# vchuravy/NewtonKrylov.jl

Measured on AMD Instinct MI355X. Metric: Krylov matvecs/sec + achieved HBM GB/s, 2D Bratu 4096^2, higher is better.
Workload: dtype f64

## Files before the change

### newtonkrylov.jl_amd/csrc/nk_resident.hip

```cpp
#include <hip/hip_runtime.h>

#include <algorithm>
#include <cmath>
#include <cstdio>
#include <vector>

#include "nk_device.hpp"

namespace nk {
namespace {
constexpr int kResMax = 64;
constexpr int kResThreads = 256;
struct ResArgs {
    const double* V[kResMax + 1];
    double* q;
    double* vout;
    double* col;
    double* colh;
    const double* red_in;
    uint64_t* gran;
    int* err;
    int noxchg;
    int ntc;
    int nwc;
    int poll1;
    int strided;
    int mirror;
    uint64_t* tstamp;
    int senders;
    const double *ju, *jv, *jf0, *jaux;
    double jeps, jlam, jhx2, jhy2;
    int64_t jnx;
    int jv_on;
    int64_t n2;
    int np, red_len, rl;
    unsigned tag0, mb0, spin;
};

template <int RV>
struct ResState {
    dx2 r[RV];
};

__device__ __forceinline__ double res_exchange(const ResArgs& A, double part, int t, double* sh, unsigned& budget,
                                              unsigned* xdone) {
    const int tid = threadIdx.x, G = gridDim.x;
    const unsigned tag = A.tag0 + (unsigned)t;
    uint64_t* slot = A.gran + (size_t)(t & 1) * G * 2;
    if (tid == 0) {
        const uint64_t bits = (uint64_t)__double_as_longlong(part);
        __hip_atomic_store(slot + 2 * blockIdx.x, ((uint64_t)tag << 32) | (bits & 0xffffffffull), __ATOMIC_RELAXED,
                           __HIP_MEMORY_SCOPE_AGENT);
        __hip_atomic_store(slot + 2 * blockIdx.x + 1, ((uint64_t)tag << 32) | (bits >> 32), __ATOMIC_RELAXED,
                           __HIP_MEMORY_SCOPE_AGENT);
    }
    if (A.poll1) {
        const int w = tid >> 6, nw = A.poll1 >= 2 ? kResThreads / 64 : 1;
        if (w < nw) {
            for (int i = 0; i < w; ++i) __builtin_amdgcn_s_sleep(8);
            const int l = tid & 63;
            uint64_t w8[8];
            bool mine = false;
            for (;;) {
                if (nw > 1 && __hip_atomic_load(xdone, __ATOMIC_RELAXED, __HIP_MEMORY_SCOPE_WORKGROUP) == tag) break;
                bool ok = true;
#pragma unroll
                for (int j = 0; j < 4; ++j) {
                    const int bl = 64 * j + l;
                    if (bl < G) {
                        w8[2 * j] = __hip_atomic_load(slot + 2 * bl, __ATOMIC_RELAXED, __HIP_MEMORY_SCOPE_AGENT);
                        w8[2 * j + 1] = __hip_atomic_load(slot + 2 * bl + 1, __ATOMIC_RELAXED, __HIP_MEMORY_SCOPE_AGENT);
                        ok = ok && (unsigned)(w8[2 * j] >> 32) == tag && (unsigned)(w8[2 * j + 1] >> 32) == tag;
                    } else {
                        w8[2 * j] = w8[2 * j + 1] = 0;
                    }
                }
                if (__all(ok)) {
                    mine = true;
                    break;
                }
                if (budget == 0 || --budget == 0) {
                    __hip_atomic_store(A.err, 1, __ATOMIC_RELAXED, __HIP_MEMORY_SCOPE_SYSTEM);
                    mine = true;
                    break;
                }
                __builtin_amdgcn_s_sleep(2);
            }
            if (mine) {
                double p = 0.0;
#pragma unroll
                for (int j = 0; j < 4; ++j)
                    p += __longlong_as_double((long long)(((w8[2 * j + 1] & 0xffffffffull) << 32) | (w8[2 * j] & 0xffffffffull)));
                p = wave_sum(p);
                if (l == 0) {
                    sh[kShB] = p;
                    if (nw > 1) __hip_atomic_store(xdone, tag, __ATOMIC_RELAXED, __HIP_MEMORY_SCOPE_WORKGROUP);
                }
            }
        }
        __syncthreads();
        const double s1 = sh[kShB];
        if (A.mb0 == 0) return s1;
        const unsigned epoch = A.mb0 + (unsigned)t;
        if ((int)blockIdx.x < A.senders) mb_send(s1, epoch);
        __syncthreads();
        return mb_recv(epoch, sh);
    }
    double v = 0.0;
    if (tid < G) {
        const uint64_t* g = slot + 2 * tid;
        uint64_t lo = __hip_atomic_load(g, __ATOMIC_RELAXED, __HIP_MEMORY_SCOPE_AGENT);
        uint64_t hi = __hip_atomic_load(g + 1, __ATOMIC_RELAXED, __HIP_MEMORY_SCOPE_AGENT);
        while ((unsigned)(lo >> 32) != tag || (unsigned)(hi >> 32) != tag) {
            if (budget == 0 || --budget == 0) {
                __hip_atomic_store(A.err, 1, __ATOMIC_RELAXED, __HIP_MEMORY_SCOPE_SYSTEM);
                lo = hi = 0;
                break;
            }
            __builtin_amdgcn_s_sleep(1);
            lo = __hip_atomic_load(g, __ATOMIC_RELAXED, __HIP_MEMORY_SCOPE_AGENT);
            hi = __hip_atomic_load(g + 1, __ATOMIC_RELAXED, __HIP_MEMORY_SCOPE_AGENT);
        }
        v = __longlong_as_double((long long)(((hi & 0xffffffffull) << 32) | (lo & 0xffffffffull)));
    }
    __syncthreads();
    double s = block_sum<kResThreads>(v, sh);
    if (tid == 0) sh[kShB] = s;
    __syncthreads();
    s = sh[kShB];
    if (A.mb0 == 0) return s;
    const unsigned epoch = A.mb0 + (unsigned)t;
    if ((int)blockIdx.x < A.senders) mb_send(s, epoch);
    __syncthreads();
    return mb_recv(epoch, sh);
}

__device__ __forceinline__ dx2 res_jv_pair(const ResArgs& A, int64_t e, double& acc) {
    const int64_t p = 2 * e, nx = A.jnx;
    const int64_t i = p % nx;
    const dx2 vc = *reinterpret_cast<const dx2*>(A.jv + p), uc = __builtin_nontemporal_load(reinterpret_cast<const dx2*>(A.ju + p));
    const dx2 vu = *reinterpret_cast<const dx2*>(A.jv + p + nx), uu = *reinterpret_cast<const dx2*>(A.ju + p + nx);
    const dx2 vd = *reinterpret_cast<const dx2*>(A.jv + p - nx), ud = *reinterpret_cast<const dx2*>(A.ju + p - nx);
    const double vl = A.jv[p - 1], ul = A.ju[p - 1], vr = A.jv[p + 2], ur = A.ju[p + 2];
    const dx2 f0 = __builtin_nontemporal_load(reinterpret_cast<const dx2*>(A.jf0 + p));
    const dx2 ax = *reinterpret_cast<const dx2*>(A.jaux + p);
    const double eps = A.jeps;
    const double c0 = uc.x + eps * vc.x, c1 = uc.y + eps * vc.y;
    const double wl = i > 0 ? ul + eps * vl : 0.0;
    const double wr = i + 2 < nx ? ur + eps * vr : 0.0;
    const double u0 = uu.x + eps * vu.x, u1 = uu.y + eps * vu.y;
    const double d0 = ud.x + eps * vd.x, d1 = ud.y + eps * vd.y;
    const double l0 = ((c1 - 2.0 * c0) + wl) / A.jhx2 + ((u0 - 2.0 * c0) + d0) / A.jhy2;
    const double l1 = ((wr - 2.0 * c1) + c0) / A.jhx2 + ((u1 - 2.0 * c1) + d1) / A.jhy2;
    const double r0 = l0 + A.jlam * nk_exp(c0), r1 = l1 + A.jlam * nk_exp(c1);
    const dx2 val{(r0 - f0.x) / eps, (r1 - f0.y) / eps};
    acc = fma(ax.x, val.x, acc);
    acc = fma(ax.y, val.y, acc);
    return val;
}

template <int NTM>
__device__ __forceinline__ dx2 ldv(const dx2* p) {
    if constexpr (NTM == 1) return *p;
    else return __builtin_nontemporal_load(p);
}
template <int NTM>
__device__ __forceinline__ dx2 ldw(const dx2* p) {
    if constexpr (NTM == 2) return __builtin_nontemporal_load(p);
    else return *p;
}
template <int NTM>
__device__ __forceinline__ dx2 ldw_s(const dx2* p, int s, int nwc) {
#ifdef NK_KBENCH
    if (NTM != 2 && s >= nwc) return __builtin_nontemporal_load(p);
#else
    (void)s;
    (void)nwc;
#endif
    return ldw<NTM>(p);
}

template <int B>
struct ResPre {
    dx2 b[B], c[B];
};
template <int RV, int B, bool PRE, int NTM = 0>
__device__ __forceinline__ void res_prefetch(const ResArgs& A, ResPre<B>& P, int t, int64_t base, int64_t ss,
                                             bool rev = false) {
    if constexpr (PRE && RV >= B) {
        const int tid = threadIdx.x;
        const int s0 = (B == 4 && rev) ? RV + A.rl - 4 : 0;
        const dx2* vb = reinterpret_cast<const dx2*>(A.V[t]) + base + tid + s0 * ss;
        const dx2* wb = reinterpret_cast<const dx2*>(A.V[t + 1 < A.np ? t + 1 : t]) + base + tid + s0 * ss;
#pragma unroll
        for (int u = 0; u < B; ++u) {
            P.b[u] = ldv<NTM>(vb + u * ss);
            P.c[u] = ldw_s<NTM>(wb + u * ss, s0 + u, A.nwc);
        }
    }
}

template <int RV, int B, bool PRE, int NTM = 0, bool NTS = false, int LB = 4>
__device__ __forceinline__ double res_pass(const ResArgs& A, ResState<RV>& S, dx2* lq, int t, double mh, int64_t lo,
                                           int64_t hi, ResPre<B>& P, int64_t base, int64_t ss, bool rev = false) {
    const int tid = threadIdx.x;
    const bool next = t + 1 < A.np;
    const dx2* vb = reinterpret_cast<const dx2*>(A.V[t]) + base + tid;
    const dx2* wb = reinterpret_cast<const dx2*>(A.V[next ? t + 1 : t]) + base + tid;
    double acc = 0.0;
    auto upd = [&](dx2& a, const dx2 b, const dx2 c) {
        a.x = fma(mh, b.x, a.x);
        a.y = fma(mh, b.y, a.y);
        const dx2 p = next ? c : a;
        acc = fma(p.x, a.x, acc);
        acc = fma(p.y, a.y, acc);
    };
    auto regs = [&] {
        constexpr int NB = (RV + B - 1) / B;
#pragma unroll
        for (int bi = 0; bi < NB; ++bi) {
            const int s0 = bi * B;
            dx2 bv[B], cv[B];
            if (PRE && RV >= B && s0 == 0 && !(B == 4 && rev)) {
#pragma unroll
                for (int u = 0; u < B; ++u) {
                    bv[u] = P.b[u];
                    cv[u] = P.c[u];
                }
            } else {
#pragma unroll
                for (int u = 0; u < B; ++u) {
                    if (s0 + u < RV) {
                        bv[u] = ldv<NTM>(vb + (s0 + u) * ss);
                        cv[u] = ldw_s<NTM>(wb + (s0 + u) * ss, s0 + u, A.nwc);
                    }
                }
            }
#pragma unroll
            for (int u = 0; u < B; ++u)
                if (s0 + u < RV) upd(S.r[s0 + u], bv[u], cv[u]);
            __builtin_amdgcn_sched_barrier(0);
        }
    };
    const dx2* vl = vb + RV * ss;
    const dx2* wl = wb + RV * ss;
    const int rl = A.rl;
    auto lds = [&] {
        auto one4 = [&](int s, bool down) {
            dx2 bv[4], cv[4];
#pragma unroll
            for (int u = 0; u < 4; ++u) {
                bv[u] = ldv<NTM>(vl + (s + u) * ss);
                cv[u] = ldw_s<NTM>(wl + (s + u) * ss, RV + s + u, A.nwc);
            }
#pragma unroll
            for (int u0 = 0; u0 < 4; ++u0) {
                const int u = down ? 3 - u0 : u0;
                dx2 a = lq[(s + u) * kResThreads + tid];
                upd(a, bv[u], cv[u]);
                lq[(s + u) * kResThreads + tid] = a;
            }
        };
        auto one = [&](int s) {
            const dx2 b = ldv<NTM>(vl + s * ss);
            const dx2 cc = ldw_s<NTM>(wl + s * ss, RV + s, A.nwc);
            dx2 a = lq[s * kResThreads + tid];
            upd(a, b, cc);
            lq[s * kResThreads + tid] = a;
        };
        auto oneB = [&](int s) {
            dx2 bv[LB], cv[LB];
#pragma unroll
            for (int u = 0; u < LB; ++u) {
                bv[u] = ldv<NTM>(vl + (s + u) * ss);
                cv[u] = ldw_s<NTM>(wl + (s + u) * ss, RV + s + u, A.nwc);
            }
#pragma unroll
            for (int u = 0; u < LB; ++u) {
                dx2 a = lq[(s + u) * kResThreads + tid];
                upd(a, bv[u], cv[u]);
                lq[(s + u) * kResThreads + tid] = a;
            }
        };
        const int r4 = rl / 4 * 4;
        if (!rev && LB != 4) {
            const int rb = rl / LB * LB;
            for (int s = 0; s < rb; s += LB) oneB(s);
            for (int s = rb; s < r4; s += 4) one4(s, false);
            for (int s = r4; s < rl; ++s) one(s);
        } else if (!rev) {
            for (int s = 0; s < r4; s += 4) one4(s, false);
            for (int s = r4; s < rl; ++s) one(s);
        } else if (PRE && B == 4 && RV >= B) {
            {
                const int s = rl - 4;
#pragma unroll
                for (int u0 = 0; u0 < 4; ++u0) {
                    const int u = 3 - u0;
                    dx2 a = lq[(s + u) * kResThreads + tid];
                    upd(a, P.b[u], P.c[u]);
                    lq[(s + u) * kResThreads + tid] = a;
                }
            }
            int s = rl - 8;
            for (; s >= 0; s -= 4) one4(s, true);
            for (s += 3; s >= 0; --s) one(s);
        } else {
            for (int s = rl - 1; s >= r4; --s) one(s);
            for (int s = r4 - 4; s >= 0; s -= 4) one4(s, true);
        }
    };
    auto stream = [&] {
        dx2* q2 = reinterpret_cast<dx2*>(A.q);
        const dx2* v2 = reinterpret_cast<const dx2*>(A.V[t]);
        const dx2* w2 = reinterpret_cast<const dx2*>(A.V[next ? t + 1 : t]);
        auto ld = [](const dx2* p) {
            if constexpr (NTS) return __builtin_nontemporal_load(p);
            else return *p;
        };
        auto st = [](dx2* p, const dx2 v) {
            if constexpr (NTS) __builtin_nontemporal_store(v, p);
            else *p = v;
        };
        int64_t e = lo + (int64_t)(RV + rl) * kResThreads + tid;
        if constexpr (NTS) {
            const int64_t hc = std::min<int64_t>(hi, e - tid + (int64_t)A.ntc * kResThreads);
            for (; e + kResThreads < hc; e += 2 * kResThreads) {
                const int64_t e1 = e + kResThreads;
                dx2 a0 = ld(q2 + e), a1 = ld(q2 + e1);
                const dx2 b0 = __builtin_nontemporal_load(v2 + e), b1 = __builtin_nontemporal_load(v2 + e1);
                const dx2 c0 = w2[e], c1 = w2[e1];
                upd(a0, b0, c0);
                upd(a1, b1, c1);
                st(q2 + e, a0);
                st(q2 + e1, a1);
            }
        }
        for (; e + kResThreads < hi; e += 2 * kResThreads) {
            const int64_t e1 = e + kResThreads;
            dx2 a0 = ld(q2 + e), a1 = ld(q2 + e1);
            const dx2 b0 = __builtin_nontemporal_load(v2 + e), b1 = __builtin_nontemporal_load(v2 + e1);
            const dx2 c0 = ld(w2 + e), c1 = ld(w2 + e1);
            upd(a0, b0, c0);
            upd(a1, b1, c1);
            st(q2 + e, a0);
            st(q2 + e1, a1);
        }
        if (e < hi) {
            dx2 a0 = ld(q2 + e);
            const dx2 b0 = __builtin_nontemporal_load(v2 + e);
            const dx2 c0 = ld(w2 + e);
            upd(a0, b0, c0);
            st(q2 + e, a0);
        }
    };
    if (rev) lds();
    regs();
    if (!rev) lds();
    stream();
    return acc;
}

template <int RV, int B = (RV > 80 ? 6 : RV > 64 ? 4 : 8), bool PRE = false, bool JV = false, bool ALT = false,
          int NTM = 0, bool NTS = false, int LB = 4>
__global__ __launch_bounds__(kResThreads, 1) void k_mgs_res(ResArgs A) {
    extern __shared__ dx2 lq[];
    __shared__ double sh[kShN];
    __shared__ unsigned xdone;
    const int tid = threadIdx.x, G = gridDim.x;
    if (tid == 0) xdone = 0;
    const int64_t ns = (A.n2 + kResThreads - 1) / kResThreads;
    const int64_t lo = (int64_t)blockIdx.x * ns / G * kResThreads;
    const int64_t hi = std::min<int64_t>((int64_t)(blockIdx.x + 1) * ns / G * kResThreads, A.n2);
    int64_t base = A.strided ? (int64_t)blockIdx.x * kResThreads : lo;
    int64_t ss = A.strided ? (int64_t)G * kResThreads : kResThreads;
#ifdef NK_KBENCH
    if (A.mirror && (blockIdx.x & 1)) {
        base = hi - kResThreads;
        ss = -(int64_t)kResThreads;
    }
#endif
    ResState<RV> S;
    ResPre<B> P;
    double h;
    unsigned budget = A.spin;
    constexpr int xo = JV ? 1 : 0;
    if constexpr (JV) {
        double jacc = 0.0;
        constexpr int kJvStage = 16;
#pragma unroll
        for (int s0 = 0; s0 < RV; s0 += kJvStage) {
            const int m = RV - s0 < kJvStage ? RV - s0 : kJvStage;
#pragma unroll 4
            for (int u = 0; u < m; ++u) lq[u * kResThreads + tid] = res_jv_pair(A, base + (s0 + u) * ss + tid, jacc);
#pragma unroll
            for (int u = 0; u < kJvStage; ++u)
                if (s0 + u < RV) S.r[s0 + u] = lq[u * kResThreads + tid];
        }
#pragma unroll 4
        for (int s = 0; s < A.rl; ++s) lq[s * kResThreads + tid] = res_jv_pair(A, base + (RV + s) * ss + tid, jacc);
        res_prefetch<RV, B, PRE, NTM>(A, P, 0, base, ss);
        h = res_exchange(A, block_sum<kResThreads>(jacc, sh), 0, sh, budget, &xdone);
    } else {
        const dx2* qb = reinterpret_cast<const dx2*>(A.q) + base + tid;
#pragma unroll
        for (int s = 0; s < RV; ++s) S.r[s] = qb[s * ss];
        for (int s = 0; s < A.rl; ++s) lq[s * kResThreads + tid] = qb[(RV + s) * ss];
        res_prefetch<RV, B, PRE, NTM>(A, P, 0, base, ss);
        h = reduce_input(A.red_in, A.red_len, sh);
    }
    for (int t = 0; t < A.np; ++t) {
        if (blockIdx.x == 0 && tid == 0) {
            A.col[t] = h;
            if (A.colh) A.colh[t] = h;
        }
        const double acc = res_pass<RV, B, PRE, NTM, NTS, LB>(A, S, lq, t, -h, lo, hi, P, base, ss, ALT && (t & 1));
        if (t + 1 < A.np) res_prefetch<RV, B, PRE, NTM>(A, P, t + 1, base, ss, ALT && ((t + 1) & 1));
        const double part = block_sum<kResThreads>(acc, sh);
#ifdef NK_KBENCH
        if (A.tstamp && tid == 0) A.tstamp[((size_t)t * G + blockIdx.x) * 2] = wall_clock64();
        if (!A.noxchg) h = res_exchange(A, part, t + xo, sh, budget, &xdone);
        else __syncthreads();
        if (A.tstamp && tid == 0) A.tstamp[((size_t)t * G + blockIdx.x) * 2 + 1] = wall_clock64();
#else
        h = res_exchange(A, part, t + xo, sh, budget, &xdone);
#endif
    }
    if (blockIdx.x == 0 && tid == 0) {
        const double r = sqrt(h);
        A.col[A.np] = r;
        if (A.colh) A.colh[A.np] = r;
    }
    if (A.vout) {
        const double hn = sqrt(h);
        dx2* vw = reinterpret_cast<dx2*>(A.vout) + base + tid;
#pragma unroll
        for (int s = 0; s < RV; ++s) vw[s * ss] = dx2{S.r[s].x / hn, S.r[s].y / hn};
        for (int s = 0; s < A.rl; ++s) {
            const dx2 a = lq[s * kResThreads + tid];
            vw[(RV + s) * ss] = dx2{a.x / hn, a.y / hn};
        }
        return;
    }
    dx2* qw = reinterpret_cast<dx2*>(A.q) + base + tid;
#pragma unroll
    for (int s = 0; s < RV; ++s) qw[s * ss] = S.r[s];
    for (int s = 0; s < A.rl; ++s) qw[(RV + s) * ss] = lq[s * kResThreads + tid];
}

template <int RV, int B = (RV > 80 ? 6 : RV > 64 ? 4 : 8), bool PRE = false, bool JV = false, bool ALT = false,
          int NTM = 0, bool NTS = false, int LB = 4>
const char* go_res(dim3 g, dim3 b, size_t lds, hipStream_t s, const ResArgs& A) {
    hipLaunchKernelGGL((k_mgs_res<RV, B, PRE, JV, ALT, NTM, NTS, LB>), g, b, lds, s, A);
    static char name[80] = {};
    if (!name[0]) {
        auto tf = [](bool x) { return x ? "true" : "false"; };
        std::snprintf(name, sizeof name, "nk::k_mgs_res<%d, %d, %s, %s, %s, %d, %s, %d>", RV, B, tf(PRE), tf(JV), tf(ALT), NTM,
                      tf(NTS), LB);
    }
    return name;
}

template <int RV, int B = (RV > 80 ? 6 : RV > 64 ? 4 : 8), bool PRE = false, bool JV = false, bool ALT = false,
          int NTM = 0, bool NTS = false, int LB = 4>
bool res_attr(size_t lds) {
    return hipFuncSetAttribute(reinterpret_cast<const void*>(&k_mgs_res<RV, B, PRE, JV, ALT, NTM, NTS, LB>),
                               hipFuncAttributeMaxDynamicSharedMemorySize, (int)lds) == hipSuccess;
}
}

hipError_t resident_bind_mb(const MbInfo& m) { return hipMemcpyToSymbol(HIP_SYMBOL(g_mb), &m, sizeof(m)); }


int launch_mgs_sweep(nk_ctx* c, int64_t n, double* q, const double* const* V, int k, int np, Red in, double* col,
                     double* colh, int rv, double** vout, const ResJv* jin) {
    if (np < 1 || np > kResMax || (n & 1) || !c->res_ok) return 1;
#ifdef NK_KBENCH
    static const int jv_env = NK_TUNE("NK_RES_JV", 0);
    if (jin && (!jv_env || !vout || !*vout || jin->nx % 2 != 0)) return 1;
#else
    if (jin) return 1;
#endif
    if (c->comm && !c->mb_on) return 1;
    if (!c->res_gran) {
        int dev = 0, cus = 0, lds = 0;
        bool ok = hipGetDevice(&dev) == hipSuccess &&
                  hipDeviceGetAttribute(&cus, hipDeviceAttributeMultiprocessorCount, dev) == hipSuccess &&
                  hipDeviceGetAttribute(&lds, hipDeviceAttributeMaxSharedMemoryPerBlock, dev) == hipSuccess &&
                  cus >= 1 && cus <= kResThreads;
        if (ok) {
            c->res_blocks = std::max(1, cus / std::max(1, c->res_share));
            const int avail = lds - (int)(sizeof(double) * kShN) - 256;
            c->res_rl = std::max(0, avail / (int)(kResThreads * sizeof(dx2)));
            const size_t lmax = (size_t)c->res_rl * kResThreads * sizeof(dx2);
            ok = res_attr<0>(lmax) && res_attr<16>(lmax) && res_attr<25>(lmax) && res_attr<32>(lmax) && res_attr<48>(lmax) &&
                 res_attr<64>(lmax) && res_attr<89, 4, true>(lmax) && res_attr<89, 4, true, false, false, 0, true>(lmax);
#ifdef NK_KBENCH
            ok = ok && res_attr<89>(lmax) && res_attr<89, 4>(lmax) && res_attr<89, 6, false, true>(lmax) &&
                 res_attr<0, 8, false, true>(lmax) && res_attr<89, 6, false, false, true>(lmax) &&
                 res_attr<89, 6, false, false, false, 1>(lmax) && res_attr<89, 6, false, false, false, 2>(lmax) &&
                 res_attr<89, 6, false, false, false, 0, true>(lmax) && res_attr<89, 2, true>(lmax) &&
                 res_attr<89, 4, true, false, false, 0, false, 8>(lmax) &&
                 res_attr<89, 4, true, false, false, 0, false, 6>(lmax) && res_attr<89, 4, true, false, true>(lmax);
#endif
            int per_cu = 0;
            ok = ok && hipOccupancyMaxActiveBlocksPerMultiprocessor(
                           &per_cu, reinterpret_cast<const void*>(&k_mgs_res<89, 4, true>), kResThreads, lmax) == hipSuccess &&
                 per_cu >= 1;
        }
        ok = ok && hipMalloc(&c->res_gran, sizeof(uint64_t) * 4 * kResThreads) == hipSuccess;
        ok = ok && hipMemsetAsync(c->res_gran, 0, sizeof(uint64_t) * 4 * kResThreads, c->stream) == hipSuccess;
        ok = ok && hipHostMalloc(&c->res_err, sizeof(int), hipHostMallocMapped) == hipSuccess;
        if (ok) *c->res_err = 0;
        ok = ok && hipHostGetDevicePointer(reinterpret_cast<void**>(&c->res_err_dev), c->res_err, 0) == hipSuccess;
        if (!ok) {
            (void)hipGetLastError();
            c->res_ok = false;
            return 1;
        }
    }
    ResArgs A{};
    for (int t = 0; t < np; ++t) A.V[t] = V[t % k];
    A.V[np] = V[(np) % k];
    A.q = q;
    A.col = col;
    A.colh = colh;
    A.red_in = in.ptr;
    A.red_len = in.len;
    A.gran = c->res_gran;
    A.err = c->res_err_dev;
    A.n2 = n >> 1;
    A.np = np;
    static const int nts_env = NK_TUNE("NK_RES_NTS", 1);
    static const int pre_env = NK_TUNE("NK_RES_PRE", 1);
    int xv = -1;
    bool streamed = false;
    {
        const int64_t G = c->res_blocks, n2 = n >> 1;
        const int64_t ns = (n2 + kResThreads - 1) / kResThreads;
        const int64_t whole = ns / G - (n2 % kResThreads != 0 ? 1 : 0);
        if (whole < 1) return 1;
        const int slots = (int)std::min<int64_t>(whole, 1 << 20);
        static const int rl_env = NK_TUNE("NK_RES_RL", -1);
        static const int rv_env = NK_TUNE("NK_RES_RV", -1);
        int rl = std::min(slots, rl_env >= 0 ? std::min(rl_env, c->res_rl) : c->res_rl);
        const bool explicit_rv = rv >= 0 || rv_env >= 0;
#ifdef NK_KBENCH
        if (rv >= 1000) {
            xv = rv - 1000;
            rv = 89;
        }
#endif
        if (rv < 0) rv = rv_env >= 0 ? rv_env : slots - rl;
        static const int kRv[] = {89, 64, 48, 32, 25, 16, 0};
        int pick = 0;
        for (int r : kRv)
            if (r <= rv && r <= slots) {
                pick = r;
                break;
            }
        if (xv < 0) rv = pick;
        else if (rv > slots) return 1;
        A.rl = std::min(rl, slots - rv);
        if (xv == 11 && A.rl < 4) xv = 0;
        const int64_t chunk = std::max<int64_t>(1, ns / G);
        const double f = (double)(rv + A.rl) / (double)chunk;
        if (!explicit_rv && (np < 2 || f < (nts_env ? 0.1 : 0.2))) return 1;
        const bool full = n2 % kResThreads == 0 && (ns + G - 1) / G <= rv + A.rl;
        streamed = !full;
        static const int vout_env = NK_TUNE("NK_RES_VOUT", 1);
        if (vout && *vout && !(full && vout_env)) *vout = nullptr;
        A.vout = vout ? *vout : nullptr;
        if (jin && (!A.vout || (rv != 0 && rv != 89) || (rv > 0 && A.rl < 16))) return 1;
        static const int strided_env = NK_TUNE("NK_RES_STRIDED", 0);
        A.strided = strided_env && n2 % kResThreads == 0 && ns % G == 0 && ns / G == rv + A.rl;
        A.mirror = NK_TUNE("NK_RES_MIRROR", 0) && !A.strided && n2 % kResThreads == 0 && ns % G == 0 && ns / G == rv + A.rl;
    }
#ifdef NK_KBENCH
    if (jin) {
        A.jv_on = 1;
        A.ju = jin->u;
        A.jv = jin->v;
        A.jf0 = jin->F0;
        A.jaux = jin->aux;
        A.jeps = jin->eps;
        A.jlam = jin->lam;
        A.jhx2 = jin->hx2;
        A.jhy2 = jin->hy2;
        A.jnx = jin->nx;
    }
#endif
    const unsigned nx_ = (unsigned)np + (jin ? 1u : 0u);
    if (c->res_tag > 0xfffffff0u - (unsigned)(kResMax + 1)) {
        NK_HIP(c, hipMemsetAsync(c->res_gran, 0, sizeof(uint64_t) * 4 * kResThreads, c->stream));
        c->res_tag = 0;
    }
    A.tag0 = c->res_tag + 1;
    c->res_tag += nx_;
    A.mb0 = 0;
    if (c->mb_on) {
        if (c->mb_epoch + nx_ > 0xffffu) c->mb_epoch = 0;
        A.mb0 = c->mb_epoch + 1;
        c->mb_epoch += nx_;
    }
#ifdef NK_KBENCH
    A.noxchg = NK_TUNE("NK_RES_NOXCHG", 0);
#endif
    static const int ntc_env = NK_TUNE("NK_RES_NTC", -1);
    static const int mall_mb = NK_TUNE("NK_RES_MALL_MB", 244);
    {
        const double slot = 4096.0 * c->res_blocks;
        const double room = 1e6 * mall_mb - slot * (rv + A.rl);
        A.ntc = ntc_env >= 0 ? ntc_env : (room > 0 ? (int)(room / slot) : 0);
    }
    A.poll1 = NK_TUNE("NK_RES_POLL1", 1);
    A.nwc = NK_TUNE("NK_RES_NWC", 1 << 30);
    A.tstamp = c->res_tstamp;
    static const int senders = NK_TUNE("NK_MB_SENDERS", 8);
    A.senders = std::max(1, std::min(senders, c->res_blocks));
    A.spin = 1u << 22;
    const size_t lds = (size_t)A.rl * kResThreads * sizeof(dx2);
    const double f = std::min(1.0, (double)c->res_blocks * (rv + A.rl) * kResThreads / (double)(n >> 1));
    const double per_res = (jin ? 5.0 : 2.0) + 2.0 * np - 1.0, per_str = 4.0 * np - 1.0;
    const double bytes = 8.0 * (double)n * (f * per_res + (1.0 - f) * per_str);
    const double dram = 8.0 * (double)n * (f * ((jin ? 5.0 : 2.0) + np) + (1.0 - f) * (3.0 * np));
    ++c->n_sweep_resident;
    const char* kn = nullptr;
    return launch_dyn(c, jin ? "arnoldi_step" : "mgs_sweep", [&] {
        const dim3 g(c->res_blocks), b(kResThreads);
        switch (rv) {
        case 0:
#ifdef NK_KBENCH
            if (jin) kn = go_res<0, 8, false, true>(g, b, lds, c->stream, A);
            else
#endif
                kn = go_res<0>(g, b, lds, c->stream, A);
            break;
        case 16: kn = go_res<16>(g, b, lds, c->stream, A); break;
        case 25: kn = go_res<25>(g, b, lds, c->stream, A); break;
        case 48: kn = go_res<48>(g, b, lds, c->stream, A); break;
        case 64: kn = go_res<64>(g, b, lds, c->stream, A); break;
        case 89:
#ifdef NK_KBENCH
            if (jin) kn = go_res<89, 6, false, true>(g, b, lds, c->stream, A);
            else if (xv == 0) kn = go_res<89, 4, true>(g, b, lds, c->stream, A);
            else if (xv == 1) kn = go_res<89, 4>(g, b, lds, c->stream, A);
            else if (xv == 2) kn = go_res<89, 6, false, false, true>(g, b, lds, c->stream, A);
            else if (xv == 3) kn = go_res<89, 6, false, false, false, 1>(g, b, lds, c->stream, A);
            else if (xv == 4) kn = go_res<89, 6, false, false, false, 2>(g, b, lds, c->stream, A);
            else if (xv == 5) kn = go_res<89, 6, false, false, false, 0, true>(g, b, lds, c->stream, A);
            else if (xv == 6) kn = go_res<89, 4, true, false, false, 0, true>(g, b, lds, c->stream, A);
            else if (xv == 8) kn = go_res<89, 2, true>(g, b, lds, c->stream, A);
            else if (xv == 9) kn = go_res<89, 4, true, false, false, 0, false, 8>(g, b, lds, c->stream, A);
            else if (xv == 10) kn = go_res<89, 4, true, false, false, 0, false, 6>(g, b, lds, c->stream, A);
            else if (xv == 11) kn = go_res<89, 4, true, false, true>(g, b, lds, c->stream, A);
            else if (streamed && nts_env && pre_env)
                kn = go_res<89, 4, true, false, false, 0, true>(g, b, lds, c->stream, A);
            else if (streamed && nts_env) kn = go_res<89, 6, false, false, false, 0, true>(g, b, lds, c->stream, A);
            else if (pre_env) kn = go_res<89, 4, true>(g, b, lds, c->stream, A);
            else kn = go_res<89>(g, b, lds, c->stream, A);
#else
            (void)xv;
            (void)pre_env;
            if (streamed) kn = go_res<89, 4, true, false, false, 0, true>(g, b, lds, c->stream, A);
            else kn = go_res<89, 4, true>(g, b, lds, c->stream, A);
#endif
            break;
        default: kn = go_res<32>(g, b, lds, c->stream, A); break;
        }
        return bytes;
    }, dram, &kn);
}

}

#ifdef NK_KBENCH
namespace nk {
namespace {
__global__ __launch_bounds__(kBlock) void k_hashfill(int64_t n, double* __restrict__ x, uint64_t seed) {
    for (int64_t i = (int64_t)blockIdx.x * kBlock + threadIdx.x; i < n; i += (int64_t)gridDim.x * kBlock) {
        uint64_t z = (uint64_t)i * 0x9e3779b97f4a7c15ull + seed;
        z = (z ^ (z >> 30)) * 0xbf58476d1ce4e5b9ull;
        z = (z ^ (z >> 27)) * 0x94d049bb133111ebull;
        z ^= z >> 31;
        x[i] = (double)(z >> 11) * 0x1.0p-53 - 0.5;
    }
}
}
}

extern "C" int nkb_mgs_res(nk_ctx* c, int64_t n, int k, int rv, int reps, double* us_out, double* us_ref, double* diff_out) {
    using namespace nk;
    if (!c || n < 2 || k < 1 || k > kResMax || reps < 1 || !us_out || !us_ref || !diff_out) return NK_E_ARG;
    const char* tsf = getenv("NK_RES_TSTAMP");
    if (tsf && *tsf && !c->res_tstamp) NK_HIP(c, hipMalloc(&c->res_tstamp, sizeof(uint64_t) * 2 * kResMax * 1024));
    std::vector<double*> V(k + 3, nullptr), Vbase(k + 3, nullptr);
    const size_t stag = (size_t)std::max(0, NK_TUNE("NK_ALLOC_STAGGER", 131072)) / 256 * 32;
    for (size_t v = 0; v < V.size(); ++v) {
        const size_t sh = (v % 8) * stag;
        NK_HIP(c, hipMalloc(&Vbase[v], sizeof(double) * (n + sh)));
        V[v] = Vbase[v] + sh;
        hipLaunchKernelGGL(k_hashfill, dim3(2048), dim3(kBlock), 0, c->stream, n, V[v], (uint64_t)(v + 1) * 7919u);
    }
    double* q0 = V[k];
    double* qa = V[k + 1];
    double* qb = V[k + 2];
    double* col = c->scal + 64;
    double* col2 = c->scal + 64 + 2 * kResMax;
    hipEvent_t e0, e1;
    NK_HIP(c, hipEventCreate(&e0));
    NK_HIP(c, hipEventCreate(&e1));
    double ms_a = 0.0, ms_b = 0.0;
    for (int r = 0; r <= reps; ++r) {
        float ms = 0.f;
        NK_TRY(launch_copy(c, n, qa, q0));
        Red red{};
        NK_TRY(launch_dot(c, n, V[0], qa, &red));
        NK_HIP(c, hipEventRecord(e0, c->stream));
        for (int t = 0; t < k; ++t) {
            Red nxt{};
            NK_TRY(launch_mgs_pass(c, n, qa, V[t], t + 1 < k ? V[t + 1] : nullptr, red, col + t, nullptr, &nxt, 0));
            red = nxt;
        }
        NK_TRY(launch_finalize(c, red, col + k, 1, nullptr));
        NK_HIP(c, hipEventRecord(e1, c->stream));
        NK_HIP(c, hipEventSynchronize(e1));
        NK_HIP(c, hipEventElapsedTime(&ms, e0, e1));
        if (r > 0) ms_a += ms;
        NK_TRY(launch_copy(c, n, qb, q0));
        NK_TRY(launch_dot(c, n, V[0], qb, &red));
        NK_HIP(c, hipEventRecord(e0, c->stream));
        const int rc = launch_mgs_sweep(c, n, qb, V.data(), k, k, red, col2, nullptr, rv, nullptr, nullptr);
        if (rc != NK_OK) return rc == 1 ? fail(c, NK_E_ARG, "resident sweep not applicable") : rc;
        NK_HIP(c, hipEventRecord(e1, c->stream));
        NK_HIP(c, hipEventSynchronize(e1));
        NK_HIP(c, hipEventElapsedTime(&ms, e0, e1));
        if (r > 0) ms_b += ms;
        if (*c->res_err) return fail(c, NK_E_HIP, "resident sweep: granule poll timed out");
    }
    *us_ref = 1e3 * ms_a / ((double)reps * k);
    *us_out = 1e3 * ms_b / ((double)reps * k);
    std::vector<double> a(n), b(n), ca(k + 1), cb(k + 1);
    NK_HIP(c, hipMemcpy(a.data(), qa, sizeof(double) * n, hipMemcpyDeviceToHost));
    NK_HIP(c, hipMemcpy(b.data(), qb, sizeof(double) * n, hipMemcpyDeviceToHost));
    NK_HIP(c, hipMemcpy(ca.data(), col, sizeof(double) * (k + 1), hipMemcpyDeviceToHost));
    NK_HIP(c, hipMemcpy(cb.data(), col2, sizeof(double) * (k + 1), hipMemcpyDeviceToHost));
    double m = 0.0, d = 0.0, dh = 0.0;
    for (int64_t i = 0; i < n; ++i) {
        m = std::max(m, std::fabs(a[i]));
        d = std::max(d, std::fabs(a[i] - b[i]));
    }
    for (int i = 0; i <= k; ++i) dh = std::max(dh, std::fabs(ca[i] - cb[i]) / std::max(1e-300, std::fabs(ca[i])));
    diff_out[0] = m > 0 ? d / m : d;
    diff_out[1] = dh;
    diff_out[2] = (double)c->res_rl;
    if (c->res_tstamp && tsf && *tsf) {
        std::vector<uint64_t> ts((size_t)2 * k * c->res_blocks);
        NK_HIP(c, hipMemcpy(ts.data(), c->res_tstamp, sizeof(uint64_t) * ts.size(), hipMemcpyDeviceToHost));
        if (FILE* f = std::fopen(tsf, "wb")) {
            std::fwrite(ts.data(), sizeof(uint64_t), ts.size(), f);
            std::fclose(f);
        }
        (void)hipFree(c->res_tstamp);
        c->res_tstamp = nullptr;
    }
    diff_out[3] = (double)c->res_blocks;
    (void)hipEventDestroy(e0);
    (void)hipEventDestroy(e1);
    for (auto p : Vbase) (void)hipFree(p);
    return NK_OK;
}
#endif
```

Before: 1274.

## Split LDS-resident tail slots into separate update and dot phases around register work

```diff
diff --git a/newtonkrylov.jl_amd/csrc/nk_resident.hip b/newtonkrylov.jl_amd/csrc/nk_resident.hip
--- a/newtonkrylov.jl_amd/csrc/nk_resident.hip
+++ b/newtonkrylov.jl_amd/csrc/nk_resident.hip
@@ -3,6 +3,7 @@
 #include <algorithm>
 #include <cmath>
 #include <cstdio>
+#include <type_traits>
 #include <vector>
 
 #include "nk_device.hpp"
@@ -11,6 +12,14 @@
 namespace {
 constexpr int kResMax = 64;
 constexpr int kResThreads = 256;
+#ifndef NK_RES_TAIL_DEFAULT
+#define NK_RES_TAIL_DEFAULT 24
+#endif
+constexpr int kResTail = NK_RES_TAIL_DEFAULT;
+#ifdef NK_KBENCH
+int g_res_tail_hook = -1;
+int g_res_tail_launched = 0;
+#endif
 struct ResArgs {
     const double* V[kResMax + 1];
     double* q;
@@ -34,6 +43,7 @@
     int jv_on;
     int64_t n2;
     int np, red_len, rl;
+    int tg;
     unsigned tag0, mb0, spin;
 };
 
@@ -245,6 +255,52 @@
     const dx2* vl = vb + RV * ss;
     const dx2* wl = wb + RV * ss;
     const int rl = A.rl;
+    const int tg = rev ? 0 : A.tg;
+    const int rf = rl - tg;
+    auto tail_upd = [&](int s, auto nb) {
+        constexpr int N = decltype(nb)::value;
+        dx2 bv[N];
+#pragma unroll
+        for (int u = 0; u < N; ++u) bv[u] = vl[(s + u) * ss];
+#pragma unroll
+        for (int u = 0; u < N; ++u) {
+            dx2 a = lq[(s + u) * kResThreads + tid];
+            a.x = fma(mh, bv[u].x, a.x);
+            a.y = fma(mh, bv[u].y, a.y);
+            lq[(s + u) * kResThreads + tid] = a;
+        }
+    };
+    auto tail_dot = [&](int s, auto nb) {
+        constexpr int N = decltype(nb)::value;
+        if (next) {
+            dx2 cv[N];
+#pragma unroll
+            for (int u = 0; u < N; ++u) cv[u] = wl[(s + u) * ss];
+#pragma unroll
+            for (int u = 0; u < N; ++u) {
+                const dx2 a = lq[(s + u) * kResThreads + tid];
+                acc = fma(cv[u].x, a.x, acc);
+                acc = fma(cv[u].y, a.y, acc);
+            }
+        } else {
+#pragma unroll
+            for (int u = 0; u < N; ++u) {
+                const dx2 a = lq[(s + u) * kResThreads + tid];
+                acc = fma(a.x, a.x, acc);
+                acc = fma(a.y, a.y, acc);
+            }
+        }
+    };
+    auto tail = [&](auto&& f) {
+        int s = rf;
+        __builtin_amdgcn_sched_barrier(0);
+        for (; s + 8 <= rl; s += 8) {
+            f(s, std::integral_constant<int, 8>{});
+            __builtin_amdgcn_sched_barrier(0);
+        }
+        for (; s < rl; ++s) f(s, std::integral_constant<int, 1>{});
+        __builtin_amdgcn_sched_barrier(0);
+    };
     auto lds = [&] {
         auto one4 = [&](int s, bool down) {
             dx2 bv[4], cv[4];
@@ -282,18 +338,18 @@
                 lq[(s + u) * kResThreads + tid] = a;
             }
         };
-        const int r4 = rl / 4 * 4;
+        const int r4 = rf / 4 * 4;
         if (!rev && LB != 4) {
-            const int rb = rl / LB * LB;
+            const int rb = rf / LB * LB;
             for (int s = 0; s < rb; s += LB) oneB(s);
             for (int s = rb; s < r4; s += 4) one4(s, false);
-            for (int s = r4; s < rl; ++s) one(s);
+            for (int s = r4; s < rf; ++s) one(s);
         } else if (!rev) {
             for (int s = 0; s < r4; s += 4) one4(s, false);
-            for (int s = r4; s < rl; ++s) one(s);
+            for (int s = r4; s < rf; ++s) one(s);
         } else if (PRE && B == 4 && RV >= B) {
             {
-                const int s = rl - 4;
+                const int s = rf - 4;
 #pragma unroll
                 for (int u0 = 0; u0 < 4; ++u0) {
                     const int u = 3 - u0;
@@ -302,11 +358,11 @@
                     lq[(s + u) * kResThreads + tid] = a;
                 }
             }
-            int s = rl - 8;
+            int s = rf - 8;
             for (; s >= 0; s -= 4) one4(s, true);
             for (s += 3; s >= 0; --s) one(s);
         } else {
-            for (int s = rl - 1; s >= r4; --s) one(s);
+            for (int s = rf - 1; s >= r4; --s) one(s);
             for (int s = r4 - 4; s >= 0; s -= 4) one4(s, true);
         }
     };
@@ -355,8 +411,10 @@
         }
     };
     if (rev) lds();
+    tail(tail_upd);
     regs();
     if (!rev) lds();
+    tail(tail_dot);
     stream();
     return acc;
 }
@@ -575,6 +633,15 @@
         static const int strided_env = NK_TUNE("NK_RES_STRIDED", 0);
         A.strided = strided_env && n2 % kResThreads == 0 && ns % G == 0 && ns / G == rv + A.rl;
         A.mirror = NK_TUNE("NK_RES_MIRROR", 0) && !A.strided && n2 % kResThreads == 0 && ns % G == 0 && ns / G == rv + A.rl;
+        static const int tail_env = NK_TUNE("NK_RES_TAIL", kResTail);
+        int tail = tail_env;
+#ifdef NK_KBENCH
+        if (g_res_tail_hook >= 0) tail = g_res_tail_hook;
+#endif
+        A.tg = full && xv != 2 && xv != 11 ? std::max(0, std::min(tail, A.rl)) : 0;
+#ifdef NK_KBENCH
+        g_res_tail_launched = A.tg;
+#endif
     }
 #ifdef NK_KBENCH
     if (jin) {
@@ -689,7 +756,8 @@
 }
 }
 
-extern "C" int nkb_mgs_res(nk_ctx* c, int64_t n, int k, int rv, int reps, double* us_out, double* us_ref, double* diff_out) {
+static int mgs_res_bench(nk_ctx* c, int64_t n, int k, int rv, int tail, int reps, double* us_out, double* us_ref,
+                         double* diff_out, double* q_out, double* col_out, int* tail_out) {
     using namespace nk;
     if (!c || n < 2 || k < 1 || k > kResMax || reps < 1 || !us_out || !us_ref || !diff_out) return NK_E_ARG;
     const char* tsf = getenv("NK_RES_TSTAMP");
@@ -730,7 +798,9 @@
         NK_TRY(launch_copy(c, n, qb, q0));
         NK_TRY(launch_dot(c, n, V[0], qb, &red));
         NK_HIP(c, hipEventRecord(e0, c->stream));
+        g_res_tail_hook = tail;
         const int rc = launch_mgs_sweep(c, n, qb, V.data(), k, k, red, col2, nullptr, rv, nullptr, nullptr);
+        g_res_tail_hook = -1;
         if (rc != NK_OK) return rc == 1 ? fail(c, NK_E_ARG, "resident sweep not applicable") : rc;
         NK_HIP(c, hipEventRecord(e1, c->stream));
         NK_HIP(c, hipEventSynchronize(e1));
@@ -754,6 +824,9 @@
     diff_out[0] = m > 0 ? d / m : d;
     diff_out[1] = dh;
     diff_out[2] = (double)c->res_rl;
+    if (tail_out) *tail_out = g_res_tail_launched;
+    if (q_out) std::copy(b.begin(), b.end(), q_out);
+    if (col_out) std::copy(cb.begin(), cb.end(), col_out);
     if (c->res_tstamp && tsf && *tsf) {
         std::vector<uint64_t> ts((size_t)2 * k * c->res_blocks);
         NK_HIP(c, hipMemcpy(ts.data(), c->res_tstamp, sizeof(uint64_t) * ts.size(), hipMemcpyDeviceToHost));
@@ -770,4 +843,16 @@
     for (auto p : Vbase) (void)hipFree(p);
     return NK_OK;
 }
-#endif
+
+extern "C" int nkb_mgs_res(nk_ctx* c, int64_t n, int k, int rv, int reps, double* us_out, double* us_ref, double* diff_out) {
+    return mgs_res_bench(c, n, k, rv, -1, reps, us_out, us_ref, diff_out, nullptr, nullptr, nullptr);
+}
+
+extern "C" int nkb_mgs_res_tail(nk_ctx* c, int64_t n, int k, int rv, int tail, int reps, double* us_out, double* us_ref,
+                                double* diff_out, double* q_out, double* col_out, int* tail_out) {
+    if (!tail_out) return NK_E_ARG;
+    return mgs_res_bench(c, n, k, rv, tail, reps, us_out, us_ref, diff_out, q_out, col_out, tail_out);
+}
+
+extern "C" int nkb_res_tail_last(void) { return nk::g_res_tail_launched; }
+#endif
```

After: 1300 (median of 6 runs). +2.1%, better.
